# boyden/NuHTC

Hardware: AMD Instinct MI355X
Metric: tiles/sec (256x256) whole-node (higher is better)
Workload: dtype f32

## Files before the change

### include/nuhtc_hip.h

```cpp
#ifndef NUHTC_HIP_H
#define NUHTC_HIP_H

#include <stddef.h>
#include <stdint.h>

#ifdef __cplusplus
extern "C" {
#endif

#define NUHTC_ABI_VERSION 12

enum {
  NUHTC_OK = 0,
  NUHTC_E_INVALID = -1,
  NUHTC_E_HIP = -2,
  NUHTC_E_STATE = -3,
  NUHTC_E_CAPACITY = -4,
  NUHTC_E_NOTFOUND = -5
};

enum { NUHTC_CH_AS_IS = 0, NUHTC_CH_SWAP = 1 };

enum { NUHTC_PIPE_BF16_SPLIT = 0, NUHTC_PIPE_FP32 = 1 };

// ... 184 lines not shown
  const int32_t* det_off;
  const int32_t* det_counts;
  int32_t B, D, max_keep, H, W, vH, vW;
  float scale, thr;
  uint32_t* masks;
  int32_t* areas;
} nuhtc_paste_args;
int nuhtc_op_paste(nuhtc_engine* e, const nuhtc_paste_args* a, void* stream);
typedef struct nuhtc_tile_post_args {
  const float* dets;
  const int32_t* labels;
  const int32_t* areas;
  const int32_t* det_counts;
  const uint32_t* masks;
  uint8_t* keep;
  int32_t B, max_keep, H, W, vH, vW, margin, min_area;
  float thr;
} nuhtc_tile_post_args;
int nuhtc_op_tile_post(nuhtc_engine* e, const nuhtc_tile_post_args* a, void* stream);
int nuhtc_op_rpn_select(nuhtc_engine* e, const float* const out[4], const int32_t h[4], const int32_t w[4], int B, int nms_pre, int img_h, int img_w,
                        float min_size, float* cand_boxes, float* cand_scores, int32_t* cand_count, void* stream);
int nuhtc_op_nms_levels(nuhtc_engine* e, const float* boxes, const float* scores, const int32_t* group_count, int B, int G, int slot, float iou_thr,
                        int max_keep, int route, float* dets, int32_t* src, int32_t* counts, void* stream);
int nuhtc_op_build_rois(nuhtc_engine* e, const float* cc_boxes, const int32_t* cc_counts, int cc_cap, const float* rpn_dets, const int32_t* rpn_counts,
                        int rpn_cap, const float* fixed, int n_fixed, int B, int cap, float* rois, int32_t* roi_off, int32_t* roi_cnt, int32_t* total,
                        void* stream);

#define NUHTC_AP_AUTO 0
#define NUHTC_AP_GEMM 1
#define NUHTC_AP_KERNEL 2
#define NUHTC_AP_FP16 3
int nuhtc_op_attn_pool(nuhtc_engine* e, const float* F, int B, int HW, float tau, int route, float* G, void* stream);
typedef struct nuhtc_roi_feats_args {
  const float* x0;
  const float* x1;
  const float* sem;
  const float* x0sem;
  const float* G2;
  const float* G3;
  const float* rois;
  const int32_t* r_dev;
  int32_t B, cap, P;
  int32_t H[4], W[4];
  float* out;
  uint8_t* fb_flag;
  int32_t* counts;
// ... 99 lines not shown
```

### nuhtc_amd/csrc/engine.h

```cpp
#pragma once
#include <unordered_map>

#include "common.h"

struct StageGeom {
  int H, W, C, nH;
  int Hp, Wp, nW;
  int* map[2];
  int* cidx[2];
  int* ctok[2];
  int* vrow[2];
  unsigned long long* padbits[2];
  int* brow;
  int bias_row;
  float* mask;
  int* mask_any;
};

enum BlockRoute { ROUTE_PLAIN, ROUTE_A_LN, ROUTE_FUSED };

struct BlockW {
  BlockRoute route;
  float *n1g, *n1b, *relbT , *qkv_w, *qkv_b, *proj_w, *proj_b, *n2g, *n2b, *f1_w, *f1_b, *f2_w, *f2_b;
  float *qkv_wln, *qkv_bln, *f1_wln, *f1_bln;
// ... 30 lines not shown
  float *lat_w[4], *lat_b[4], *fpn_w[4], *fpn_b[4];
  float *rpn_w, *rpn_b, *rpn_hw, *rpn_hb;
  void *rpn_hf, *sem_lf[4], *sem_ef;
  float *sem_lw[4], *sem_lb[4], *sem_cw[4], *sem_cb[4], *sem_ew, *sem_eb, *sem_gw, *sem_gb;
  float *fc1_w[3], *fc1_b[3], *fc2_w[3], *fc2_b[3], *head_w[3], *head_b[3];
  float *mk_w[4], *mk_b[4], *mk_up_w, *mk_up_b, *mk_lw, *mk_lb;

  float *img, *tokA, *tokB, *xw, *qkv, *att, *hid;
  float* tok[4] = {};
  float* ln_out[4] = {};
  float *lat_wln[4] = {}, *lat_bln[4] = {};
  const uint8_t* in_tiles = nullptr;
  int in_swap = 0;
  int last_batch = 0;
  float* ln_part2 = nullptr;
  float* ln_part = nullptr;
  float *c[4], *lat[4], *x[4], *rpn[4], *semg[4];
  float *tmpA, *tmpB, *tmpR, *sem_feat, *sem_pred, *x0sem;
  PoolLevels pool{};
  double* pool_slab = nullptr;
  int roi_cap = 0;
  int cand_cap = 0;
  int* overflow = nullptr;
  int* overflow_host = nullptr;
  int32_t* export_pos = nullptr;
  int32_t* crop_size = nullptr;
  hipStream_t own = nullptr;
  hipStream_t side = nullptr;
  hipEvent_t ev_rpn = nullptr, ev_side = nullptr, ev_fpn = nullptr;
  hipStream_t side2 = nullptr;
  hipEvent_t ev_side2 = nullptr;
  struct RoiWs* rw = nullptr;
};

int dev_alloc(nuhtc_engine* e, void** p, size_t bytes);
int upload_bytes(nuhtc_engine* e, void** dst, const void* host, size_t bytes);
template <typename T>
int upload(nuhtc_engine* e, T** dst, const std::vector<T>& v) {
  return upload_bytes(e, (void**)dst, v.data(), v.size() * sizeof(T));
}
template <typename T>
int ws(nuhtc_engine* e, T** p, const char* name, std::vector<int64_t> shape, int dtype) {
  size_t n = 1;
  for (auto d : shape) n *= (size_t)d;
  int rc = dev_alloc(e, (void**)p, n * sizeof(T));
  if (rc) return rc;
// ... 32 lines not shown
```

### nuhtc_amd/csrc/proposals.h

```cpp
#pragma once
#include "common.h"

#define NMS_MAX_CAP 16384
#define NMS_MAX_GROUPS 16
#define CC_LIST_CAP 4096

struct RpnLevels {
  const float* out[4];
  int h[4], w[4], stride[4];
};

struct RpnSelParams {
  int nms_pre;
  int slot;
  float* cand_boxes;
  float* cand_scores;
  int* cand_count;
  int img_h, img_w;
  float min_size;
  unsigned* keys;
  int key_stride;
};

struct NmsParams {
  const float* boxes;
  const float* scores;
// ... 13 lines not shown
  int* out_counts;
  int* seg_start;
  int* seg_n;
  int* sorted_pos;
  unsigned long long* keepbits;
};

struct CcParams {
  const float* sem_pred;
  int h, w, img_h, img_w;
  int min_area, cap;
  unsigned char *mask_a, *mask_b, *touch;
  int* labels;
  int* stats;
  int* list;
  int* nlist;
  float* boxes;
  int* counts;
  int* overflow;
};

int launch_rpn_select(const RpnLevels& lv, const RpnSelParams& p, int B, hipStream_t s);
int launch_nms(const NmsParams& p, int B, hipStream_t s);
int launch_nms_levels(const NmsParams& p, int B, hipStream_t s);
int nms_set_attributes();
int launch_cc_mask(const CcParams& p, int B, hipStream_t s);
int launch_cc_from_mask(const CcParams& p, int B, bool open, hipStream_t s);
int launch_cc_proposals(const CcParams& p, int B, hipStream_t s);
```

### nuhtc_amd/csrc/proposals.hip

```cpp
#include "block_prims.h"
#include "common.h"
#include "proposals.h"

typedef unsigned long long u64;

__global__ __launch_bounds__(1024) void rpn_level_kernel(RpnLevels lv, RpnSelParams p) {
  __shared__ u64 keys[4096];
  __shared__ int hist[256];
  __shared__ int sc16[17];
  __shared__ unsigned s_prefix;
  __shared__ int s_need, s_cnt, s_eq;
  const int b = blockIdx.x, L = blockIdx.y;
  const int tid = threadIdx.x;
  const int h = lv.h[L], w = lv.w[L], stride = lv.stride[L];
  const int n = h * w * 3;
  const float* out = lv.out[L] + (long long)b * h * w * 32;
  const int k = p.nms_pre;
  auto score_of = [&](int idx) -> float {
    int pix = idx / 3, a = idx - pix * 3;
    float x = out[(long long)pix * 32 + a];
    return 1.0f / (1.0f + expf(-x));
  };
  int nsel;
  constexpr int RPN_KPT = 48;
// ... 459 lines not shown
  const u64* kb = p.keepbits + (long long)b * nw;
  for (int idx = tid; idx < nchunks * 64; idx += 1024) {
    if ((kb[idx >> 6] >> (idx & 63)) & 1ull) {
      const long long a = (long long)b * p.cap + idx;
      const float sc = p.scores[p.sorted_src[a]];
      const int k = atomicAdd(&s_n, 1);
      if (k < 8192) keys[k] = ((u64)desc_key_nonneg(sc) << 32) | ((u64)(unsigned)p.sorted_pos[a] << 16) | (unsigned)idx;
    }
  }
  __syncthreads();
  const int n = min(s_n, 8192);
  const int npad = next_pow2(n < 2 ? 2 : n);
  for (int i = n + tid; i < npad; i += 1024) keys[i] = ~0ull;
  __syncthreads();
  bitonic_sort_u64<1024>(keys, npad, tid);
  const int nout = min(n, p.max_keep);
  for (int k = tid; k < nout; k += 1024) {
    const int idx = (int)(keys[k] & 0xFFFFu);
    emit_det(p, b, k, p.sorted_src[(long long)b * p.cap + idx]);
  }
  if (tid == 0) p.out_counts[b] = nout;
}

int launch_nms_levels(const NmsParams& p, int B, hipStream_t s) {
  DEV_SKIP(128);
  ProfScope ps("nms", 0, 0, s);
  if (p.cap % 64 || p.cap > NMS_MAX_CAP + 64 * NMS_MAX_GROUPS || p.cap >= 65536 || p.n_groups > NMS_MAX_GROUPS || p.ids ||
      p.n_groups * p.max_keep > 8192 || !p.seg_start || !p.seg_n || !p.sorted_pos || !p.keepbits)
    return NUHTC_E_INVALID;
  size_t lds = (size_t)next_pow2(p.slot < 2 ? 2 : p.slot) * sizeof(u64);
  hipLaunchKernelGGL(nms_prepare_levels_kernel, dim3(B, p.n_groups), dim3(1024), lds, s, p);
  const int slot_chunks = (p.slot + 63) / 64;
  hipLaunchKernelGGL(nms_mask_levels_kernel, dim3(cdiv(p.n_groups * (slot_chunks * (slot_chunks + 1) / 2), 4), 1, B), dim3(256), 0, s, p);
  hipLaunchKernelGGL(nms_reduce_levels_kernel, dim3(B, p.n_groups), dim3(256), 0, s, p);
  hipLaunchKernelGGL(nms_select_kernel, dim3(B), dim3(1024), 0, s, p);
  return launched() ? 0 : NUHTC_E_HIP;
}

int nms_set_attributes() {
  hipError_t e = hipFuncSetAttribute((const void*)nms_prepare_kernel, hipFuncAttributeMaxDynamicSharedMemorySize, NMS_MAX_CAP * 8);
  if (e == hipSuccess)
    e = hipFuncSetAttribute((const void*)nms_prepare_levels_kernel, hipFuncAttributeMaxDynamicSharedMemorySize, NMS_MAX_CAP * 8);
  return e == hipSuccess ? 0 : NUHTC_E_HIP;
}

struct Gauss5 { float k[25]; };

constexpr int CCM_TW = 64, CCM_TH = 32;
__global__ __launch_bounds__(256) void cc_mask_kernel(const float* __restrict__ pred, unsigned char* __restrict__ m, int h, int w, int H,
                                                      int W, Gauss5 gk) {
  __shared__ float up[CCM_TH + 4][CCM_TW + 4 + 1];
  const int b = blockIdx.z;
  const int X0 = blockIdx.x * CCM_TW, Y0 = blockIdx.y * CCM_TH;
  const float* pb = pred + (long long)b * h * w;
  const float sy = h > 1 ? (float)(h - 1) / (float)(H - 1) : 0.f;
  const float sx = w > 1 ? (float)(w - 1) / (float)(W - 1) : 0.f;
  constexpr int NE = (CCM_TH + 4) * (CCM_TW + 4);
#pragma unroll 2
  for (int e = threadIdx.x; e < NE; e += 256) {
    int ly = e / (CCM_TW + 4), lx = e - ly * (CCM_TW + 4);
    int Y = Y0 + ly - 2, X = X0 + lx - 2;
    if (Y < 0) Y = -Y; if (Y >= H) Y = 2 * H - 2 - Y;
    if (X < 0) X = -X; if (X >= W) X = 2 * W - 2 - X;
    Y = Y < 0 ? 0 : Y; X = X < 0 ? 0 : X;
    float fy = sy * Y, fx = sx * X;
// ... 292 lines not shown
```

### nuhtc_amd/csrc/roi_engine.hip

```cpp
#include <cmath>
#include <cstring>

#include "engine.h"
#include "proposals.h"
#include "roi.h"

#define BIG_SPLIT_MAX 512
struct RoiWs {
  float *cand_boxes, *cand_scores;
  unsigned* rpn_keys;
  int rpn_key_stride;
  int* cand_count;
  float *nms_sboxes;
  int *nms_src, *nms_ntotal, *nms_seg_start, *nms_seg_n, *nms_pos;
  unsigned long long* nms_keepbits;
  unsigned long long* nms_mask;
  float* rpn_dets;
  int *rpn_src, *rpn_counts;
  int rpn_slot, rpn_cap, rpn_pow2;
  unsigned char *cc_a, *cc_b, *cc_touch;
  int *cc_labels, *cc_stats, *cc_counts, *cc_list, *cc_nlist;
  float* cc_boxes;
  float* rois;
  int *roi_off, *roi_cnt, *roi_total;
  float *G2, *G3, *ap_inv, *ap_S, *ap_Ft;
  float *feats, *h1, *h2;
  int *fb_count, *fb_list, *mid_list;
  float* big_part;
  unsigned char* fb_flag;
  float *cls[3], *reg[3];
  int total_cap;
  float *dc_boxes, *dc_scores;
  int *dc_ids, *dc_count;
  int det_cap, det_pow2;
  float* det_dets;
  int *det_src, *det_counts, *det_labels;
  float* mask_rois;
  int *det_off, *det_total;
  float *mfeat, *mtmpA, *mtmpB, *mup, *mprob;
  int mask_cap;
  unsigned* masks_own;
  int* areas_own;
// ... 58 lines not shown

static int round_up(int v, int m) { return (v + m - 1) / m * m; }
static int pow2_ge(int v) { int p = 2; while (p < v) p <<= 1; return p; }

int alloc_roi_workspace(nuhtc_engine* e) {
  const nuhtc_config& c = e->cfg;
  const int B = c.max_batch;
  const int Hn = e->Hn, Wn = e->Wn;
  RoiWs* w = new RoiWs();
  memset(w, 0, sizeof(*w));
  e->rw = w;
  int rc;
  if ((rc = nms_set_attributes())) { e->err = "hipFuncSetAttribute(nms_prepare) failed"; return rc; }
  w->rpn_slot = c.rpn_nms_pre;
  int maxc = 0;
  for (int l = 0; l < 4; ++l) maxc += std::min(c.rpn_nms_pre, e->st[l].H * e->st[l].W * 3);
  w->rpn_cap = round_up(std::max(maxc, 64), 64) + 64 * 3;
  w->rpn_pow2 = pow2_ge(maxc);
  e->roi_cap = c.max_cc_proposals + c.rpn_max_per_img;
  w->det_cap = round_up(e->roi_cap * c.num_classes, 64);
  w->det_pow2 = pow2_ge(e->roi_cap * c.num_classes);
  if (maxc > NMS_MAX_CAP || w->det_cap > NMS_MAX_CAP) { e->err = "candidate capacity exceeds NMS_MAX_CAP (reduce rpn_nms_pre / max_cc_proposals)"; return NUHTC_E_INVALID; }
  const int nmscap = std::max(w->rpn_cap, w->det_cap);
  w->rpn_key_stride = round_up(e->st[0].H * e->st[0].W * 3, 64);
  if ((rc = ws(e, &w->rpn_keys, nullptr, {B, 4, w->rpn_key_stride}, 1)) ||
      (rc = ws(e, &w->cand_boxes, "rpn_cand_boxes", {B, 4, w->rpn_slot, 4}, 0)) || (rc = ws(e, &w->cand_scores, "rpn_cand_scores", {B, 4, w->rpn_slot}, 0)) ||
      (rc = ws(e, &w->cand_count, "rpn_cand_count", {B, 4}, 1)) || (rc = ws(e, &w->nms_sboxes, nullptr, {B, nmscap, 4}, 0)) ||
      (rc = ws(e, &w->nms_src, nullptr, {B, nmscap}, 1)) || (rc = ws(e, &w->nms_ntotal, nullptr, {B}, 1)) ||
      (rc = ws(e, &w->nms_seg_start, nullptr, {B, 4}, 1)) || (rc = ws(e, &w->nms_seg_n, nullptr, {B, 4}, 1)) ||
      (rc = ws(e, &w->nms_pos, nullptr, {B, nmscap}, 1)) || (rc = ws(e, &w->nms_keepbits, nullptr, {B, nmscap / 64}, 3)) ||
      (rc = ws(e, &w->nms_mask, nullptr, {B, nmscap, nmscap / 64}, 3)) || (rc = ws(e, &w->rpn_dets, "rpn_props", {B, c.rpn_max_per_img, 5}, 0)) ||
      (rc = ws(e, &w->rpn_src, nullptr, {B, c.rpn_max_per_img}, 1)) || (rc = ws(e, &w->rpn_counts, "rpn_counts", {B}, 1)))
    return rc;
  const int64_t HW = (int64_t)Hn * Wn;
  const int ccc = std::max(c.max_cc_proposals, 1);
  if ((rc = ws(e, &w->cc_a, nullptr, {B, HW}, 2)) || (rc = ws(e, &w->cc_b, "cc_mask", {B, Hn, Wn}, 2)) || (rc = ws(e, &w->cc_touch, nullptr, {B, HW}, 2)) ||
      (rc = ws(e, &w->cc_labels, "cc_labels", {B, Hn, Wn}, 1)) || (rc = ws(e, &w->cc_stats, nullptr, {B, HW, 5}, 1)) ||
      (rc = ws(e, &w->cc_list, nullptr, {B, CC_LIST_CAP}, 1)) || (rc = ws(e, &w->cc_nlist, nullptr, {B}, 1)) ||
      (rc = ws(e, &w->cc_boxes, "cc_props", {B, ccc, 4}, 0)) || (rc = ws(e, &w->cc_counts, "cc_counts", {B}, 1)) ||
      (rc = ws(e, &e->overflow, nullptr, {4}, 1)))
    return rc;
  w->total_cap = B * e->roi_cap;
  const int T = w->total_cap;
  if ((rc = ws(e, &w->rois, "rois", {T, 5}, 0)) || (rc = ws(e, &w->roi_off, "roi_off", {B}, 1)) || (rc = ws(e, &w->roi_cnt, "roi_counts", {B}, 1)) ||
      (rc = ws(e, &w->roi_total, "roi_total", {1}, 1)) || (rc = ws(e, &w->G2, "G2", {B, e->st[2].H * e->st[2].W, 64}, 0)) ||
      (rc = ws(e, &w->G3, "G3", {B, e->st[3].H * e->st[3].W, 64}, 0)) || (rc = ws(e, &w->feats, "bbox_feats", {T, 49, 64}, 0)) ||
      (rc = ws(e, &w->h1, nullptr, {T, 256}, 0)) || (rc = ws(e, &w->h2, "h2", {T, 256}, 0)) ||
      (rc = ws(e, &w->ap_inv, nullptr, {B, e->st[2].H * e->st[2].W}, 0)) ||
      (rc = ws(e, &w->ap_S, nullptr, {B, (int64_t)e->st[2].H * e->st[2].W, (int64_t)e->st[2].H * e->st[2].W}, 0)) ||
      (rc = ws(e, &w->ap_Ft, nullptr, {B, 64, e->st[2].H * e->st[2].W}, 0)) ||
      (rc = ws(e, &w->fb_count, "roi_fallback_count", {8}, 1)) || (rc = ws(e, &w->mid_list, nullptr, {T}, 1)) || (rc = ws(e, &w->fb_list, nullptr, {T}, 1)) || (rc = ws(e, &w->fb_flag, nullptr, {T}, 2)))
    return rc;
  if ((rc = ws(e, &w->big_part, nullptr, {BIG_SPLIT_MAX, 3, 49, 64}, 0))) return rc;
  for (int k = 0; k < 3; ++k) {
// ... 50 lines not shown
}

int run_roi_path(nuhtc_engine* e, int B, const float* rois_fixed, int n_rois, int n_dets, hipStream_t s, const nuhtc_dets* out) {
  const nuhtc_config& c = e->cfg;
  RoiWs* w = e->rw;
  const int Hn = e->Hn, Wn = e->Wn;
  const bool fixed = rois_fixed != nullptr;
  if (!out || !out->boxes || !out->labels || !out->counts) FAIL(e, NUHTC_E_INVALID, "nuhtc_dets.boxes/labels/counts are required");
  if (hipMemsetAsync(e->overflow, 0, 16, s) != hipSuccess) FAIL(e, NUHTC_E_HIP, "hipMemsetAsync failed");

  if (!fixed) {
    RpnLevels lv;
    for (int l = 0; l < 4; ++l) { lv.out[l] = e->rpn[l]; lv.h[l] = e->st[l].H; lv.w[l] = e->st[l].W; lv.stride[l] = 4 << l; }
    RpnSelParams sp;
    sp.nms_pre = c.rpn_nms_pre; sp.slot = w->rpn_slot; sp.cand_boxes = w->cand_boxes; sp.cand_scores = w->cand_scores; sp.cand_count = w->cand_count; sp.keys = w->rpn_keys; sp.key_stride = w->rpn_key_stride;
    sp.img_h = e->Hv; sp.img_w = e->Wv; sp.min_size = c.rpn_min_bbox_size;
    hipStream_t s2 = e->cfg.schedule == NUHTC_SCHED_THROUGHPUT ? s : e->side;
    if (s2 != s && hipStreamWaitEvent(s2, e->ev_rpn, 0) != hipSuccess) FAIL(e, NUHTC_E_HIP, "hipStreamWaitEvent failed");
    RUN(launch_rpn_select(lv, sp, B, s2));
    NmsParams np;
    memset(&np, 0, sizeof(np));
    np.boxes = w->cand_boxes; np.scores = w->cand_scores; np.ids = nullptr; np.group_count = w->cand_count; np.n_groups = 4; np.slot = w->rpn_slot;
    np.cap = w->rpn_cap; np.cap_pow2 = w->rpn_pow2; np.iou_thr = c.rpn_nms_iou; np.max_keep = c.rpn_max_per_img;
    np.sorted_boxes = w->nms_sboxes; np.sorted_src = w->nms_src; np.n_total = w->nms_ntotal; np.mask = w->nms_mask;
    np.out_dets = w->rpn_dets; np.out_src = w->rpn_src; np.out_counts = w->rpn_counts;
    np.seg_start = w->nms_seg_start; np.seg_n = w->nms_seg_n; np.sorted_pos = w->nms_pos; np.keepbits = w->nms_keepbits;
    RUN(launch_nms_levels(np, B, s2));
    if (s2 != s && hipEventRecord(e->ev_side, s2) != hipSuccess) FAIL(e, NUHTC_E_HIP, "hipEventRecord failed");
    if (c.watershed_proposal && c.max_cc_proposals > 0) {
      CcParams cp;
      cp.sem_pred = e->sem_pred; cp.h = e->st[0].H; cp.w = e->st[0].W; cp.img_h = e->Hv; cp.img_w = e->Wv; cp.min_area = 10;    cp.cap = c.max_cc_proposals;
      cp.mask_a = w->cc_a; cp.mask_b = w->cc_b; cp.touch = w->cc_touch; cp.labels = w->cc_labels; cp.stats = w->cc_stats; cp.boxes = w->cc_boxes;
      cp.counts = w->cc_counts; cp.overflow = e->overflow; cp.list = w->cc_list; cp.nlist = w->cc_nlist;
      RUN(launch_cc_proposals(cp, B, s));
    }
  }
  const bool use_cc = !fixed && c.watershed_proposal && c.max_cc_proposals > 0;
  for (int l = 2; l < 4; ++l)
    RUN(attn_pool_table(e, e->x[l], l == 2 ? w->G2 : w->G3, B, e->st[l].H * e->st[l].W, c.att_thres, NUHTC_AP_AUTO, w->ap_inv, w->ap_S, w->ap_Ft, s));
  if (e->cfg.schedule != NUHTC_SCHED_THROUGHPUT && hipStreamWaitEvent(s, fixed ? e->ev_rpn : e->ev_side, 0) != hipSuccess) FAIL(e, NUHTC_E_HIP, "hipStreamWaitEvent failed");
  RUN(launch_build_rois(use_cc ? w->cc_boxes : nullptr, w->cc_counts, std::max(c.max_cc_proposals, 1), w->rpn_dets, w->rpn_counts, c.rpn_max_per_img,
                        rois_fixed, n_rois, w->rois, w->roi_off, w->roi_cnt, w->roi_total, B, s));
  const int Rcap = fixed ? B * n_rois : B * e->roi_cap;

  RoiFeatParams fp;
  fp.rois = w->rois; fp.r_dev = w->roi_total; fp.x0 = e->x[0]; fp.x1 = e->x[1]; fp.G2 = w->G2; fp.G3 = w->G3; fp.sem = e->sem_feat; fp.x0sem = e->x0sem;
  fp.H0 = e->st[0].H; fp.W0 = e->st[0].W; fp.H1 = e->st[1].H; fp.W1 = e->st[1].W; fp.H2 = e->st[2].H; fp.W2 = e->st[2].W; fp.H3 = e->st[3].H; fp.W3 = e->st[3].W;
// ... 259 lines not shown
  int maxn = 0;
  for (int l = 0; l < 4; ++l) {
    if (h[l] < 1 || w[l] < 1 || (long long)h[l] * w[l] * 3 > (1ll << 24)) FAIL(e, NUHTC_E_INVALID, "rpn_select op: level size out of range");
    maxn = std::max(maxn, h[l] * w[l] * 3);
  }
  HIP_CHECK(e, hipSetDevice(e->device));
  hipStream_t s = (hipStream_t)stream;
  RpnLevels lv;
  for (int l = 0; l < 4; ++l) { lv.out[l] = out[l]; lv.h[l] = h[l]; lv.w[l] = w[l]; lv.stride[l] = 4 << l; }
  DevScratch sc;
  RpnSelParams sp;
  sp.nms_pre = nms_pre; sp.slot = nms_pre; sp.cand_boxes = cand_boxes; sp.cand_scores = cand_scores; sp.cand_count = cand_count;
  sp.key_stride = round_up(maxn, 64);
  sp.keys = sc.alloc<unsigned>((size_t)B * 4 * sp.key_stride * sizeof(unsigned));
  sp.img_h = img_h; sp.img_w = img_w; sp.min_size = min_size;
  if (!sc.ok()) FAIL(e, NUHTC_E_HIP, "rpn_select op: scratch allocation failed");
  const int rc = launch_rpn_select(lv, sp, B, s);
  return op_finish(e, rc, s, "rpn_select launch refused or failed", "rpn_select kernel failed");
}

int nuhtc_op_nms_levels(nuhtc_engine* e, const float* boxes, const float* scores, const int32_t* group_count, int B, int G, int slot, float iou_thr,
                        int max_keep, int route, float* dets, int32_t* src, int32_t* counts, void* stream) {
  if (!e || !boxes || !scores || !group_count || !dets || !src || !counts) return NUHTC_E_INVALID;
  if (!e->finalized) FAIL(e, NUHTC_E_STATE, "nuhtc_op_nms_levels before finalize");
  if (B < 1 || B > 256) FAIL(e, NUHTC_E_INVALID, "nms_levels op: B out of range (1..256)");
  if (G < 1 || G > NMS_MAX_GROUPS || slot < 1 || slot > NMS_MAX_CAP || max_keep < 1 || (route != 0 && route != 1))
    FAIL(e, NUHTC_E_INVALID, "nms_levels op: G (1..16), slot (1..16384), max_keep (>= 1) or route (0, 1) out of range");
  HIP_CHECK(e, hipSetDevice(e->device));
  hipStream_t s = (hipStream_t)stream;
  std::vector<int> cnt;
  if (!read_ints(group_count, B * G, cnt, s)) FAIL(e, NUHTC_E_HIP, "nms_levels op: reading group_count failed");
  for (int c : cnt)
    if (c < 0 || c > slot) FAIL(e, NUHTC_E_INVALID, "nms_levels op: a group count exceeds slot");
  const int maxc = G * slot;
  const int cap = round_up(std::max(maxc, 64), 64) + 64 * (G - 1);
  const size_t nw = (size_t)cap / 64;
  if ((unsigned long long)B * cap * nw * 8 > (1ull << 32)) FAIL(e, NUHTC_E_INVALID, "nms_levels op: the mask matrix of this call would exceed 4 GiB");
  DevScratch sc;
  NmsParams np;
  memset(&np, 0, sizeof(np));
  np.boxes = boxes; np.scores = scores; np.ids = nullptr; np.group_count = group_count; np.n_groups = G; np.slot = slot;
  np.cap = cap; np.cap_pow2 = pow2_ge(maxc); np.iou_thr = iou_thr; np.max_keep = max_keep;
  np.out_dets = dets; np.out_src = src; np.out_counts = counts;
  struct { void** p; size_t bytes; } parts[] = {
      {(void**)&np.sorted_boxes, (size_t)B * cap * 16}, {(void**)&np.sorted_src, (size_t)B * cap * 4}, {(void**)&np.n_total, (size_t)B * 4},
      {(void**)&np.seg_start, (size_t)B * G * 4},       {(void**)&np.seg_n, (size_t)B * G * 4},        {(void**)&np.sorted_pos, (size_t)B * cap * 4},
      {(void**)&np.keepbits, (size_t)B * nw * 8},       {(void**)&np.mask, (size_t)B * cap * nw * 8}};
  int rc = 0;
  for (auto& part : parts) {
    *part.p = sc.alloc<void>(part.bytes);
    if (!sc.ok()) FAIL(e, NUHTC_E_HIP, "nms_levels op: scratch allocation failed");
    if (hipMemsetAsync(*part.p, 0xFF, part.bytes, s) != hipSuccess) rc = NUHTC_E_HIP;
  }
  if (!rc) rc = route == 0 ? launch_nms_levels(np, B, s) : launch_nms(np, B, s);
  return op_finish(e, rc, s, "nms_levels launch refused or failed (route 0: G * max_keep <= 8192; sorted-list capacity within the route's limit)",
                   "nms_levels kernel failed");
}

int nuhtc_op_build_rois(nuhtc_engine* e, const float* cc_boxes, const int32_t* cc_counts, int cc_cap, const float* rpn_dets, const int32_t* rpn_counts,
                        int rpn_cap, const float* fixed, int n_fixed, int B, int cap, float* rois, int32_t* roi_off, int32_t* roi_cnt, int32_t* total,
                        void* stream) {
  if (!e || !rois || !roi_off || !roi_cnt || !total) return NUHTC_E_INVALID;
  if (!fixed && (!rpn_dets || !rpn_counts || (cc_boxes && !cc_counts))) return NUHTC_E_INVALID;
  if (B < 1 || B > 256) FAIL(e, NUHTC_E_INVALID, "build_rois op: B out of range (1..256)");
  if (cap < 0 || cc_cap < 0 || rpn_cap < 0 || n_fixed < 0) FAIL(e, NUHTC_E_INVALID, "build_rois op: negative capacity");
  HIP_CHECK(e, hipSetDevice(e->device));
  hipStream_t s = (hipStream_t)stream;
  long long rows = (long long)B * n_fixed;
  if (!fixed) {
    std::vector<int> nr, ncc(B, 0);
    if (!read_ints(rpn_counts, B, nr, s) || (cc_boxes && !read_ints(cc_counts, B, ncc, s))) FAIL(e, NUHTC_E_HIP, "build_rois op: reading the counts failed");
    rows = 0;
    for (int b = 0; b < B; ++b) {
      if (nr[b] < 0 || nr[b] > rpn_cap || ncc[b] < 0 || ncc[b] > cc_cap) FAIL(e, NUHTC_E_INVALID, "build_rois op: a count exceeds its capacity");
      rows += nr[b] + ncc[b];
    }
  }
  if (rows > cap) FAIL(e, NUHTC_E_INVALID, "build_rois op: more rows than cap");
  const int rc = launch_build_rois(cc_boxes, cc_counts, cc_cap, rpn_dets, rpn_counts, rpn_cap, fixed, n_fixed, rois, roi_off, roi_cnt, total, B, s);
  return op_finish(e, rc, s, "build_rois launch failed", "build_rois kernel failed");
// ... 67 lines not shown
```

### nuhtc_amd/engine.py

```python
import ctypes
import os
import sys

import numpy as np
import torch

from . import hip


class HipError(RuntimeError):
    pass


class _DevView:

    def __init__(self, ptr, shape, typestr):
        self.__cuda_array_interface__ = dict(shape=tuple(int(s) for s in shape), typestr=typestr, data=(int(ptr), False),
                                             version=2, strides=None)


_TYPESTR = {0: '<f4', 1: '<i4', 2: '|u1', 3: '<u4'}
_TORCH = {0: torch.float32, 1: torch.int32, 2: torch.uint8, 3: torch.int32}


# ... 557 lines not shown
        hs = (ctypes.c_int32 * 4)(*[int(m.shape[1]) for m in maps])
        ws = (ctypes.c_int32 * 4)(*[int(m.shape[2]) for m in maps])
        self._check(self.lib.nuhtc_op_rpn_select(self.h, ptrs, hs, ws, B, K, int(img_hw[0]), int(img_hw[1]), float(min_size), cand_boxes.data_ptr(),
                                                 cand_scores.data_ptr(), cand_count.data_ptr(), self._stream()))
        return cand_boxes, cand_scores, cand_count

    def op_nms_levels(self, boxes, scores, counts, iou_thr, max_keep, route=0, dets=None, src=None):
        B, G, slot = (int(v) for v in scores.shape)
        if tuple(boxes.shape) != (B, G, slot, 4):
            raise ValueError('op_nms_levels: boxes (B, G, slot, 4) and scores (B, G, slot) expected')
        cnt = self._i32(np.asarray(counts).reshape(-1) if not isinstance(counts, torch.Tensor) else counts)
        if cnt.numel() != B * G:
            raise ValueError('op_nms_levels: counts (B, G) expected')
        K = int(max_keep)
        if dets is None:
            dets = torch.zeros(B, max(K, 1), 5, dtype=torch.float32, device=self.device)
        if src is None:
            src = torch.zeros(B, max(K, 1), dtype=torch.int32, device=self.device)
        out_counts = torch.zeros(B, dtype=torch.int32, device=self.device)
        self._check(self.lib.nuhtc_op_nms_levels(self.h, boxes.contiguous().data_ptr(), scores.contiguous().data_ptr(), cnt.contiguous().data_ptr(), B, G, slot,
                                                 float(iou_thr), K, int(route), dets.data_ptr(), src.data_ptr(), out_counts.data_ptr(), self._stream()))
        return dets, src, out_counts

    def op_build_rois(self, rpn_dets=None, rpn_counts=None, cc_boxes=None, cc_counts=None, fixed=None, B=None, rois=None, cap=None):
        dev = dict(dtype=torch.int32, device=self.device)
        if fixed is not None:
            B, nf = int(fixed.shape[0]), int(fixed.shape[1])
            need = B * nf
        else:
            B, nf = int(rpn_dets.shape[0]), 0
            rpn_counts = self._i32(rpn_counts)
            need = B * int(rpn_dets.shape[1])
            if cc_boxes is not None:
                cc_counts = self._i32(cc_counts)
                need += B * int(cc_boxes.shape[1])
        if rois is None:
            rois = torch.zeros(max(need if cap is None else int(cap), 1), 5, dtype=torch.float32, device=self.device)
        cap = int(rois.shape[0]) if cap is None else int(cap)
        r = dict(rois=rois, roi_off=torch.zeros(B, **dev), roi_cnt=torch.zeros(B, **dev), total=torch.zeros(1, **dev))
        ptr = lambda t: t.data_ptr() if t is not None else None
        self._check(self.lib.nuhtc_op_build_rois(self.h, ptr(cc_boxes), ptr(cc_counts), int(cc_boxes.shape[1]) if cc_boxes is not None else 1,
                                                 ptr(rpn_dets), ptr(rpn_counts), int(rpn_dets.shape[1]) if rpn_dets is not None else 1,
                                                 ptr(fixed), nf, B, cap, rois.data_ptr(), r['roi_off'].data_ptr(), r['roi_cnt'].data_ptr(),
                                                 r['total'].data_ptr(), self._stream()))
        return r

# ... 239 lines not shown
```

### nuhtc_amd/hip.py

```python
import ctypes
import os

HERE = os.path.dirname(os.path.abspath(__file__))
LIB_PATH = os.path.join(HERE, 'libnuhtc_hip.so')

RLE_MAX_RUNS = 15360
ABI_VERSION = 12

OK, E_INVALID, E_HIP, E_STATE, E_CAPACITY, E_NOTFOUND = 0, -1, -2, -3, -4, -5
CH_AS_IS, CH_SWAP = 0, 1
OVERLAP_MASK, OVERLAP_POLYGON = 0, 1
PIPE_BF16_SPLIT, PIPE_FP32 = 0, 1
ORDER_TOKEN, ORDER_COMPACT = 0, 1
SCHED_LATENCY, SCHED_THROUGHPUT = 0, 1
EVAL_PANNUKE, EVAL_CONIC = 0, 1
TISSUE_ALL, TISSUE_MEDIAN, TISSUE_THRESHOLD = 0, 1, 2


class Config(ctypes.Structure):
    _fields_ = [
        ('abi_version', ctypes.c_int32), ('num_classes', ctypes.c_int32),
        ('tile_h', ctypes.c_int32), ('tile_w', ctypes.c_int32), ('valid_h', ctypes.c_int32), ('valid_w', ctypes.c_int32), ('max_batch', ctypes.c_int32),
        ('scale_factor', ctypes.c_float), ('mean', ctypes.c_float * 3), ('std', ctypes.c_float * 3),
        ('rpn_nms_pre', ctypes.c_int32), ('rpn_max_per_img', ctypes.c_int32),
# ... 91 lines not shown
    ]


class StitchStore(ctypes.Structure):
    _fields_ = [
        ('n_img', ctypes.c_int32), ('cand_cap', ctypes.c_int32), ('pool_cap', ctypes.c_int32), ('work_cap', ctypes.c_int32),
        ('box', ctypes.c_void_p), ('area', ctypes.c_void_p), ('score', ctypes.c_void_p), ('label', ctypes.c_void_p), ('key', ctypes.c_void_p),
        ('off', ctypes.c_void_p), ('pool', ctypes.c_void_p), ('counters', ctypes.c_void_p), ('work', ctypes.c_void_p),
    ]


class Dets(ctypes.Structure):
    _fields_ = [('boxes', ctypes.c_void_p), ('labels', ctypes.c_void_p), ('counts', ctypes.c_void_p),
                ('masks', ctypes.c_void_p), ('areas', ctypes.c_void_p), ('keep', ctypes.c_void_p)]


EXPORTS = ['nuhtc_default_config', 'nuhtc_create', 'nuhtc_destroy', 'nuhtc_last_error', 'nuhtc_load_weight',
           'nuhtc_finalize', 'nuhtc_infer', 'nuhtc_infer_fixed_load', 'nuhtc_check', 'nuhtc_get_buffer',
           'nuhtc_op_gemm', 'nuhtc_op_gemm_split', 'nuhtc_op_roi_align', 'nuhtc_op_nms', 'nuhtc_profile_enable', 'nuhtc_profile_read', 'nuhtc_dev_knob', 'nuhtc_export_crops',
           'nuhtc_mask_contours', 'nuhtc_merge_overlap', 'nuhtc_export_kept', 'nuhtc_clock_probe', 'nuhtc_op_swin_mlp', 'nuhtc_stream', 'nuhtc_op_swin_proj_mlp', 'nuhtc_bind_host_thread',
           'nuhtc_bind_host_thread_pci', 'nuhtc_bind_host_thread_at', 'nuhtc_restore_host_thread', 'nuhtc_op_ln_gemm', 'nuhtc_op_gemm_ln_gemm', 'nuhtc_op_merge_ln_gemm', 'nuhtc_write_ring_features',
           'nuhtc_write_point_features', 'nuhtc_join_features', 'nuhtc_fill_rings', 'nuhtc_features', 'nuhtc_op_cc_mask', 'nuhtc_op_cc_proposals',
           'nuhtc_op_conv3', 'nuhtc_op_window_msa', 'nuhtc_op_bbox_tail', 'nuhtc_op_det_post', 'nuhtc_op_paste', 'nuhtc_op_tile_post',
           'nuhtc_op_rpn_select', 'nuhtc_op_nms_levels', 'nuhtc_op_build_rois', 'nuhtc_op_attn_pool', 'nuhtc_op_roi_feats',
           'nuhtc_eval_batch', 'nuhtc_op_eval_select', 'nuhtc_op_eval_pairs', 'nuhtc_op_eval_render', 'nuhtc_op_eval_joint',
           'nuhtc_stitch_gather', 'nuhtc_stitch_pairs', 'nuhtc_stitch_render', 'nuhtc_op_stitch_gather', 'nuhtc_op_stitch_pairs', 'nuhtc_op_stitch_render',
           'nuhtc_tissue_mask', 'nuhtc_points_polygon_test', 'nuhtc_grid_in_contour', 'nuhtc_rle_encode']

_lib = None


def load():
    global _lib
    if _lib is not None:
        return _lib
    if not os.path.exists(LIB_PATH):
        raise ImportError(f'{LIB_PATH} not found: the HIP extension is required (no CPU fallback exists). '
                          'Build it with `python -m nuhtc_amd.build` (hipcc, --offload-arch=gfx950).')
    import torch
    lib = ctypes.CDLL(LIB_PATH)
    vp, ci, cf = ctypes.c_void_p, ctypes.c_int, ctypes.c_float
    lib.nuhtc_default_config.argtypes = [ctypes.POINTER(Config)]
    lib.nuhtc_default_config.restype = None
    lib.nuhtc_create.argtypes = [ctypes.POINTER(Config), ci, ctypes.POINTER(vp)]
    lib.nuhtc_destroy.argtypes = [vp]
    lib.nuhtc_destroy.restype = None
    lib.nuhtc_last_error.argtypes = [vp]
# ... 6 lines not shown
    lib.nuhtc_check.argtypes = [vp, vp]
    lib.nuhtc_get_buffer.argtypes = [vp, ctypes.c_char_p, ctypes.POINTER(vp), ctypes.POINTER(ctypes.c_int64),
                                     ctypes.POINTER(ci), ctypes.POINTER(ci)]
    lib.nuhtc_op_gemm.argtypes = [vp, vp, vp, vp, vp, ci, ci, ci, ci, vp]
    lib.nuhtc_op_gemm_split.argtypes = [vp, vp, vp, vp, vp, vp, ci, ci, ci, ci, vp]
    lib.nuhtc_op_ln_gemm.argtypes = [vp, vp, ci, vp, vp, vp, vp, vp, vp, ci, ci, ci, ci, vp]
    lib.nuhtc_op_gemm_ln_gemm.argtypes = [vp, vp, vp, vp, vp, vp, vp, vp, vp, vp, vp, vp, ci, ci, ci, ci, ci, vp]
    lib.nuhtc_op_merge_ln_gemm.argtypes = [vp, vp, ci, ci, ci, ci, vp, vp, vp, vp, vp]
    lib.nuhtc_op_swin_mlp.argtypes = [vp, vp, vp, vp, vp, vp, vp, vp, vp, ci, ci, vp]
    lib.nuhtc_op_swin_proj_mlp.argtypes = [vp, vp, vp, vp, vp, vp, vp, vp, vp, vp, vp, vp, ci, ci, vp]
    lib.nuhtc_op_roi_align.argtypes = [vp, vp, ci, ci, ci, vp, ci, ci, cf, ci, vp, vp]
    lib.nuhtc_op_nms.argtypes = [vp, vp, vp, ci, cf, vp, vp, vp]
    lib.nuhtc_op_cc_mask.argtypes = [vp, vp, ci, ci, ci, ci, ci, vp, vp]
    lib.nuhtc_op_cc_proposals.argtypes = [vp, vp, ci, ci, ci, ci, ci, ci, vp, vp, vp, vp, vp, vp, vp, vp]
    lib.nuhtc_op_conv3.argtypes = [vp, ctypes.POINTER(Conv3Args), vp]
    lib.nuhtc_op_window_msa.argtypes = [vp, ctypes.POINTER(WmsaArgs), vp]
    lib.nuhtc_op_bbox_tail.argtypes = [vp, ctypes.POINTER(BboxTailArgs), vp]
    lib.nuhtc_op_det_post.argtypes = [vp, ctypes.POINTER(DetPostArgs), vp]
    lib.nuhtc_op_paste.argtypes = [vp, ctypes.POINTER(PasteArgs), vp]
    lib.nuhtc_op_tile_post.argtypes = [vp, ctypes.POINTER(TilePostArgs), vp]
    i4 = ctypes.POINTER(ctypes.c_int32)
    lib.nuhtc_op_rpn_select.argtypes = [vp, ctypes.POINTER(vp), i4, i4, ci, ci, ci, ci, cf, vp, vp, vp, vp]
    lib.nuhtc_op_nms_levels.argtypes = [vp, vp, vp, vp, ci, ci, ci, cf, ci, ci, vp, vp, vp, vp]
    lib.nuhtc_op_build_rois.argtypes = [vp, vp, vp, ci, vp, vp, ci, vp, ci, ci, ci, vp, vp, vp, vp, vp]
    lib.nuhtc_op_attn_pool.argtypes = [vp, vp, ci, ci, cf, ci, vp, vp]
    lib.nuhtc_op_roi_feats.argtypes = [vp, ctypes.POINTER(RoiFeatsArgs), vp]
    lib.nuhtc_eval_batch.argtypes = [vp, ctypes.POINTER(Dets), ci, ctypes.POINTER(EvalArgs), vp]
    lib.nuhtc_op_eval_select.argtypes = [vp, vp, ci, vp, vp, vp, ci, ci, ci, ci, cf, ctypes.c_double, vp, vp, vp, vp]
    lib.nuhtc_op_eval_pairs.argtypes = [vp, vp, vp, vp, vp, ci, ci, ci, ci, ci, ci, ci, vp, vp, vp, vp, vp]
    lib.nuhtc_op_eval_render.argtypes = [vp, vp, vp, vp, vp, ci, ci, ci, ci, ci, ci, vp, vp]
    lib.nuhtc_op_eval_joint.argtypes = [vp, vp, ci, vp, ci, ci, ci, ci, ci, ci, vp, vp, vp]
    sst = ctypes.POINTER(StitchStore)
    lib.nuhtc_stitch_gather.argtypes = [vp, ctypes.POINTER(Dets), ci, vp, cf, cf, sst, vp]
    lib.nuhtc_op_stitch_gather.argtypes = [vp, vp, vp, vp, vp, vp, ci, ci, ci, ci, cf, cf, sst, vp]
    lib.nuhtc_stitch_pairs.argtypes = lib.nuhtc_op_stitch_pairs.argtypes = [vp, sst, ci, vp, ci, vp, ci, ci, ci, ci, vp, vp, vp, vp]
    lib.nuhtc_stitch_render.argtypes = lib.nuhtc_op_stitch_render.argtypes = [vp, sst, ci, vp, ci, ci, ci, vp, vp, vp, vp]
    lib.nuhtc_mask_contours.argtypes = [vp, ctypes.POINTER(Dets), ci, ci, vp, vp, vp]
    lib.nuhtc_merge_overlap.argtypes = [ci, vp, vp, vp, vp, vp, ctypes.c_int64, ctypes.c_int64, ci, ctypes.c_double, ci, ci, ci, ci, vp, vp]
    lib.nuhtc_tissue_mask.argtypes = [ci, vp, ci, ci, ctypes.c_int64, ci, ci, ci, ci, ci, ci, vp, vp, vp, vp, vp]
    lib.nuhtc_points_polygon_test.argtypes = [ci, vp, ctypes.c_int64, vp, ctypes.c_int64, vp, vp]
    lib.nuhtc_grid_in_contour.argtypes = [ci, ci, ci, ci, ci, ci, vp, ci, ci, vp, ctypes.c_int64, vp, ctypes.c_int64, vp, ci, ci, ci, vp, vp]
    lib.nuhtc_rle_encode.argtypes = [ci, vp, vp, ci, ci, ci, ci, vp, vp, vp, ctypes.c_int64, vp, vp]
    lib.nuhtc_export_kept.argtypes = [vp, ctypes.POINTER(Dets), ci, vp, vp, ci, ci, vp, vp, vp, vp, vp, vp, vp, vp]
    lib.nuhtc_export_crops.argtypes = [vp, vp, vp, ci, vp, vp, vp, vp, ci, vp]
    lib.nuhtc_profile_enable.argtypes = [ci]
    lib.nuhtc_clock_probe.argtypes = [ci, ctypes.c_uint64, vp, vp]
# ... 101 lines not shown
```

Measured before the change: 2015.

## Fuse per-level RPN NMS into one LDS-resident kernel without global IoU mask

Adds a fused per-(image, level) NMS kernel for slots up to 4096. It sorts scores in LDS, builds only the 64x64 diagonal IoU bitmasks, and runs greedy suppression with on-the-fly IoU against the kept boxes. This replaces the separate prepare, mask and reduce kernels and drops the large global NMS mask allocation for the RPN path. The cost is a large LDS footprint per block, which limits occupancy, and a serial chunk loop with a block barrier per chunk.

```diff
diff --git a/include/nuhtc_hip.h b/include/nuhtc_hip.h
--- a/include/nuhtc_hip.h
+++ b/include/nuhtc_hip.h
@@ -230,6 +230,7 @@
                         float min_size, float* cand_boxes, float* cand_scores, int32_t* cand_count, void* stream);
 int nuhtc_op_nms_levels(nuhtc_engine* e, const float* boxes, const float* scores, const int32_t* group_count, int B, int G, int slot, float iou_thr,
                         int max_keep, int route, float* dets, int32_t* src, int32_t* counts, void* stream);
+int nuhtc_op_nms_levels_fused(nuhtc_engine* e);
 int nuhtc_op_build_rois(nuhtc_engine* e, const float* cc_boxes, const int32_t* cc_counts, int cc_cap, const float* rpn_dets, const int32_t* rpn_counts,
                         int rpn_cap, const float* fixed, int n_fixed, int B, int cap, float* rois, int32_t* roi_off, int32_t* roi_cnt, int32_t* total,
                         void* stream);
diff --git a/nuhtc_amd/csrc/engine.h b/nuhtc_amd/csrc/engine.h
--- a/nuhtc_amd/csrc/engine.h
+++ b/nuhtc_amd/csrc/engine.h
@@ -76,6 +76,7 @@
   int roi_cap = 0;
   int cand_cap = 0;
   int* overflow = nullptr;
+  int op_nms_fused = -1;
   int* overflow_host = nullptr;
   int32_t* export_pos = nullptr;
   int32_t* crop_size = nullptr;
diff --git a/nuhtc_amd/csrc/proposals.h b/nuhtc_amd/csrc/proposals.h
--- a/nuhtc_amd/csrc/proposals.h
+++ b/nuhtc_amd/csrc/proposals.h
@@ -2,6 +2,7 @@
 #include "common.h"
 
 #define NMS_MAX_CAP 16384
+#define NMS_FUSED_MAX_SLOT 4096
 #define NMS_MAX_GROUPS 16
 #define CC_LIST_CAP 4096
 
@@ -61,7 +62,8 @@
 
 int launch_rpn_select(const RpnLevels& lv, const RpnSelParams& p, int B, hipStream_t s);
 int launch_nms(const NmsParams& p, int B, hipStream_t s);
-int launch_nms_levels(const NmsParams& p, int B, hipStream_t s);
+bool nms_levels_fused(const NmsParams& p);
+int launch_nms_levels(const NmsParams& p, int B, hipStream_t s, int* fused = nullptr);
 int nms_set_attributes();
 int launch_cc_mask(const CcParams& p, int B, hipStream_t s);
 int launch_cc_from_mask(const CcParams& p, int B, bool open, hipStream_t s);
diff --git a/nuhtc_amd/csrc/proposals.hip b/nuhtc_amd/csrc/proposals.hip
--- a/nuhtc_amd/csrc/proposals.hip
+++ b/nuhtc_amd/csrc/proposals.hip
@@ -505,12 +505,124 @@
   if (tid == 0) p.out_counts[b] = nout;
 }
 
-int launch_nms_levels(const NmsParams& p, int B, hipStream_t s) {
+__host__ __device__ __forceinline__ int nms_fused_key_words(int slot) {
+  const int p2 = next_pow2(slot < 2 ? 2 : slot), s64 = (slot + 63) & ~63;
+  return p2 > s64 ? p2 : s64;
+}
+static size_t nms_fused_lds_bytes(int slot) { return (size_t)((slot + 63) & ~63) * 20 + (size_t)nms_fused_key_words(slot) * 8; }
+
+__global__ __launch_bounds__(1024) void nms_levels_fused_kernel(NmsParams p) {
+  extern __shared__ float4 sbox[];
+  __shared__ u64 removed[NMS_FUSED_MAX_SLOT / 64];
+  __shared__ u64 s_keep;
+  const int b = blockIdx.x, g = blockIdx.y, tid = threadIdx.x, lane = tid & 63, wave = tid >> 6;
+  const int slot64 = (p.slot + 63) & ~63;
+  u64* keys = reinterpret_cast<u64*>(sbox + slot64);
+  float* sarea = reinterpret_cast<float*>(keys + nms_fused_key_words(p.slot));
+  int goff[NMS_MAX_GROUPS + 1];
+  const float off = (float)g * (group_offsets_and_max(p, b, goff) + 1.0f);
+  int astart = 0, aend = 0;
+  for (int h = 0; h < p.n_groups; ++h) {
+    const int rows = (goff[h + 1] - goff[h] + 63) & ~63;
+    if (h < g) astart += rows;
+    aend += rows;
+  }
+  const int cnt = goff[g + 1] - goff[g];
+  const int npad = next_pow2(cnt < 2 ? 2 : cnt);
+  const long long base = (long long)(b * p.n_groups + g) * p.slot;
+  for (int i = tid; i < npad; i += 1024) keys[i] = i < cnt ? (((u64)desc_key_nonneg(p.scores[base + i])) << 32 | (unsigned)i) : ~0ull;
+  __syncthreads();
+  bitonic_sort_u64<1024>(keys, npad, tid);
+  for (int r = tid; r < cnt; r += 1024) {
+    const int i = (int)(keys[r] & 0xFFFFFFFFu);
+    const long long src = base + i;
+    const float* bx = p.boxes + src * 4;
+    const long long a = (long long)b * p.cap + astart + r;
+    const float4 o = make_float4(bx[0] + off, bx[1] + off, bx[2] + off, bx[3] + off);
+    sbox[r] = o;
+    sarea[r] = (o.z - o.x) * (o.w - o.y);
+    p.sorted_src[a] = (int)src;
+    p.sorted_pos[a] = goff[g] + i;
+  }
+  if (tid == 0) {
+    p.seg_start[b * p.n_groups + g] = astart;
+    p.seg_n[b * p.n_groups + g] = cnt;
+    if (g == 0) p.n_total[b] = aend;
+  }
+  const int nchunks = (cnt + 63) >> 6;
+  for (int i = tid; i < nchunks; i += 1024) removed[i] = 0;
+  __syncthreads();
+  u64* diag = keys;
+  for (int c = wave; c < nchunks; c += 16) {
+    const int ncol = min(cnt - c * 64, 64);
+    const int row = c * 64 + lane;
+    const bool live = lane < ncol;
+    const float4 a = sbox[live ? row : cnt - 1];
+    const float sa = sarea[live ? row : cnt - 1];
+    u64 bits = 0;
+    for (int j = 1; j < ncol; ++j) {
+      const float4 cj = sbox[c * 64 + j];
+      const float inter = box_inter(a, cj);
+      const bool mine = live && j > lane;
+      if (__ballot(mine && inter > 0.f) == 0) continue;
+      if (mine && inter_overlaps(inter, sa, sarea[c * 64 + j], p.iou_thr)) bits |= 1ull << j;
+    }
+    diag[row] = bits;
+  }
+  __syncthreads();
+  u64* kb_out = p.keepbits + (long long)b * (p.cap / 64) + astart / 64;
+  int kept = 0;
+  for (int c = 0; c < nchunks; ++c) {
+    if (kept >= p.max_keep) {
+      for (int i = c + tid; i < nchunks; i += 1024) kb_out[i] = 0;
+      break;
+    }
+    if (wave == 0) {
+      const u64 keep = greedy_chunk64(diag[c * 64 + lane], removed[c], p.max_keep - kept, cnt - c * 64);
+      if (lane == 0) { s_keep = keep; kb_out[c] = keep; }
+    }
+    __syncthreads();
+    const u64 keep = (u64)__builtin_amdgcn_readfirstlane((unsigned)(s_keep >> 32)) << 32 | (unsigned)__builtin_amdgcn_readfirstlane((unsigned)s_keep);
+    kept += __popcll(keep);
+    for (int w = c + 1 + wave; w < nchunks; w += 16) {
+      const int col = w * 64 + lane;
+      const u64 was = removed[w];
+      bool open = col < cnt && !((was >> lane) & 1ull);
+      const float4 cb = sbox[open ? col : w * 64];
+      const float ca = sarea[open ? col : w * 64];
+      bool hit = false;
+      u64 kb = keep;
+      while (kb && __ballot(open)) {
+        const int i = c * 64 + __ffsll((long long)kb) - 1;
+        kb &= kb - 1;
+        const float4 a = sbox[i];
+        const float inter = box_inter(a, cb);
+        const bool cand = open && inter > 0.f;
+        if (__ballot(cand) == 0) continue;
+        if (cand && inter_overlaps(inter, sarea[i], ca, p.iou_thr)) { hit = true; open = false; }
+      }
+      const u64 m = __ballot(hit);
+      if (lane == 0 && m) removed[w] = was | m;
+    }
+    __syncthreads();
+  }
+}
+
+bool nms_levels_fused(const NmsParams& p) { return p.slot <= NMS_FUSED_MAX_SLOT; }
+
+int launch_nms_levels(const NmsParams& p, int B, hipStream_t s, int* fused) {
   DEV_SKIP(128);
   ProfScope ps("nms", 0, 0, s);
   if (p.cap % 64 || p.cap > NMS_MAX_CAP + 64 * NMS_MAX_GROUPS || p.cap >= 65536 || p.n_groups > NMS_MAX_GROUPS || p.ids ||
       p.n_groups * p.max_keep > 8192 || !p.seg_start || !p.seg_n || !p.sorted_pos || !p.keepbits)
     return NUHTC_E_INVALID;
+  if (fused) *fused = nms_levels_fused(p);
+  if (nms_levels_fused(p)) {
+    hipLaunchKernelGGL(nms_levels_fused_kernel, dim3(B, p.n_groups), dim3(1024), nms_fused_lds_bytes(p.slot), s, p);
+    hipLaunchKernelGGL(nms_select_kernel, dim3(B), dim3(1024), 0, s, p);
+    return launched() ? 0 : NUHTC_E_HIP;
+  }
+  if (!p.sorted_boxes || !p.mask) return NUHTC_E_INVALID;
   size_t lds = (size_t)next_pow2(p.slot < 2 ? 2 : p.slot) * sizeof(u64);
   hipLaunchKernelGGL(nms_prepare_levels_kernel, dim3(B, p.n_groups), dim3(1024), lds, s, p);
   const int slot_chunks = (p.slot + 63) / 64;
@@ -524,6 +636,8 @@
   hipError_t e = hipFuncSetAttribute((const void*)nms_prepare_kernel, hipFuncAttributeMaxDynamicSharedMemorySize, NMS_MAX_CAP * 8);
   if (e == hipSuccess)
     e = hipFuncSetAttribute((const void*)nms_prepare_levels_kernel, hipFuncAttributeMaxDynamicSharedMemorySize, NMS_MAX_CAP * 8);
+  if (e == hipSuccess)
+    e = hipFuncSetAttribute((const void*)nms_levels_fused_kernel, hipFuncAttributeMaxDynamicSharedMemorySize, (int)nms_fused_lds_bytes(NMS_FUSED_MAX_SLOT));
   return e == hipSuccess ? 0 : NUHTC_E_HIP;
 }
 
diff --git a/nuhtc_amd/csrc/roi_engine.hip b/nuhtc_amd/csrc/roi_engine.hip
--- a/nuhtc_amd/csrc/roi_engine.hip
+++ b/nuhtc_amd/csrc/roi_engine.hip
@@ -18,6 +18,7 @@
   float* rpn_dets;
   int *rpn_src, *rpn_counts;
   int rpn_slot, rpn_cap, rpn_pow2;
+  bool rpn_fused;
   unsigned char *cc_a, *cc_b, *cc_touch;
   int *cc_labels, *cc_stats, *cc_counts, *cc_list, *cc_nlist;
   float* cc_boxes;
@@ -122,6 +123,11 @@
   w->det_pow2 = pow2_ge(e->roi_cap * c.num_classes);
   if (maxc > NMS_MAX_CAP || w->det_cap > NMS_MAX_CAP) { e->err = "candidate capacity exceeds NMS_MAX_CAP (reduce rpn_nms_pre / max_cc_proposals)"; return NUHTC_E_INVALID; }
   const int nmscap = std::max(w->rpn_cap, w->det_cap);
+  NmsParams rp;
+  memset(&rp, 0, sizeof(rp));
+  rp.slot = w->rpn_slot;
+  w->rpn_fused = nms_levels_fused(rp);
+  const int maskcap = w->rpn_fused ? w->det_cap : nmscap;
   w->rpn_key_stride = round_up(e->st[0].H * e->st[0].W * 3, 64);
   if ((rc = ws(e, &w->rpn_keys, nullptr, {B, 4, w->rpn_key_stride}, 1)) ||
       (rc = ws(e, &w->cand_boxes, "rpn_cand_boxes", {B, 4, w->rpn_slot, 4}, 0)) || (rc = ws(e, &w->cand_scores, "rpn_cand_scores", {B, 4, w->rpn_slot}, 0)) ||
@@ -129,7 +135,7 @@
       (rc = ws(e, &w->nms_src, nullptr, {B, nmscap}, 1)) || (rc = ws(e, &w->nms_ntotal, nullptr, {B}, 1)) ||
       (rc = ws(e, &w->nms_seg_start, nullptr, {B, 4}, 1)) || (rc = ws(e, &w->nms_seg_n, nullptr, {B, 4}, 1)) ||
       (rc = ws(e, &w->nms_pos, nullptr, {B, nmscap}, 1)) || (rc = ws(e, &w->nms_keepbits, nullptr, {B, nmscap / 64}, 3)) ||
-      (rc = ws(e, &w->nms_mask, nullptr, {B, nmscap, nmscap / 64}, 3)) || (rc = ws(e, &w->rpn_dets, "rpn_props", {B, c.rpn_max_per_img, 5}, 0)) ||
+      (rc = ws(e, &w->nms_mask, nullptr, {B, maskcap, maskcap / 64}, 3)) || (rc = ws(e, &w->rpn_dets, "rpn_props", {B, c.rpn_max_per_img, 5}, 0)) ||
       (rc = ws(e, &w->rpn_src, nullptr, {B, c.rpn_max_per_img}, 1)) || (rc = ws(e, &w->rpn_counts, "rpn_counts", {B}, 1)))
     return rc;
   const int64_t HW = (int64_t)Hn * Wn;
@@ -226,7 +232,7 @@
     memset(&np, 0, sizeof(np));
     np.boxes = w->cand_boxes; np.scores = w->cand_scores; np.ids = nullptr; np.group_count = w->cand_count; np.n_groups = 4; np.slot = w->rpn_slot;
     np.cap = w->rpn_cap; np.cap_pow2 = w->rpn_pow2; np.iou_thr = c.rpn_nms_iou; np.max_keep = c.rpn_max_per_img;
-    np.sorted_boxes = w->nms_sboxes; np.sorted_src = w->nms_src; np.n_total = w->nms_ntotal; np.mask = w->nms_mask;
+    np.sorted_boxes = w->nms_sboxes; np.sorted_src = w->nms_src; np.n_total = w->nms_ntotal; np.mask = w->rpn_fused ? nullptr : w->nms_mask;
     np.out_dets = w->rpn_dets; np.out_src = w->rpn_src; np.out_counts = w->rpn_counts;
     np.seg_start = w->nms_seg_start; np.seg_n = w->nms_seg_n; np.sorted_pos = w->nms_pos; np.keepbits = w->nms_keepbits;
     RUN(launch_nms_levels(np, B, s2));
@@ -532,6 +538,7 @@
 int nuhtc_op_nms_levels(nuhtc_engine* e, const float* boxes, const float* scores, const int32_t* group_count, int B, int G, int slot, float iou_thr,
                         int max_keep, int route, float* dets, int32_t* src, int32_t* counts, void* stream) {
   if (!e || !boxes || !scores || !group_count || !dets || !src || !counts) return NUHTC_E_INVALID;
+  e->op_nms_fused = -1;
   if (!e->finalized) FAIL(e, NUHTC_E_STATE, "nuhtc_op_nms_levels before finalize");
   if (B < 1 || B > 256) FAIL(e, NUHTC_E_INVALID, "nms_levels op: B out of range (1..256)");
   if (G < 1 || G > NMS_MAX_GROUPS || slot < 1 || slot > NMS_MAX_CAP || max_keep < 1 || (route != 0 && route != 1))
@@ -552,20 +559,24 @@
   np.boxes = boxes; np.scores = scores; np.ids = nullptr; np.group_count = group_count; np.n_groups = G; np.slot = slot;
   np.cap = cap; np.cap_pow2 = pow2_ge(maxc); np.iou_thr = iou_thr; np.max_keep = max_keep;
   np.out_dets = dets; np.out_src = src; np.out_counts = counts;
+  const bool no_mask = route == 0 && nms_levels_fused(np);
   struct { void** p; size_t bytes; } parts[] = {
       {(void**)&np.sorted_boxes, (size_t)B * cap * 16}, {(void**)&np.sorted_src, (size_t)B * cap * 4}, {(void**)&np.n_total, (size_t)B * 4},
       {(void**)&np.seg_start, (size_t)B * G * 4},       {(void**)&np.seg_n, (size_t)B * G * 4},        {(void**)&np.sorted_pos, (size_t)B * cap * 4},
       {(void**)&np.keepbits, (size_t)B * nw * 8},       {(void**)&np.mask, (size_t)B * cap * nw * 8}};
   int rc = 0;
   for (auto& part : parts) {
+    if (no_mask && part.p == (void**)&np.mask) continue;
     *part.p = sc.alloc<void>(part.bytes);
     if (!sc.ok()) FAIL(e, NUHTC_E_HIP, "nms_levels op: scratch allocation failed");
     if (hipMemsetAsync(*part.p, 0xFF, part.bytes, s) != hipSuccess) rc = NUHTC_E_HIP;
   }
-  if (!rc) rc = route == 0 ? launch_nms_levels(np, B, s) : launch_nms(np, B, s);
+  if (!rc) rc = route == 0 ? launch_nms_levels(np, B, s, &e->op_nms_fused) : launch_nms(np, B, s);
   return op_finish(e, rc, s, "nms_levels launch refused or failed (route 0: G * max_keep <= 8192; sorted-list capacity within the route's limit)",
                    "nms_levels kernel failed");
 }
+
+int nuhtc_op_nms_levels_fused(nuhtc_engine* e) { return e ? e->op_nms_fused : -1; }
 
 int nuhtc_op_build_rois(nuhtc_engine* e, const float* cc_boxes, const int32_t* cc_counts, int cc_cap, const float* rpn_dets, const int32_t* rpn_counts,
                         int rpn_cap, const float* fixed, int n_fixed, int B, int cap, float* rois, int32_t* roi_off, int32_t* roi_cnt, int32_t* total,
diff --git a/nuhtc_amd/engine.py b/nuhtc_amd/engine.py
--- a/nuhtc_amd/engine.py
+++ b/nuhtc_amd/engine.py
@@ -603,6 +603,9 @@
                                                  float(iou_thr), K, int(route), dets.data_ptr(), src.data_ptr(), out_counts.data_ptr(), self._stream()))
         return dets, src, out_counts
 
+    def op_nms_levels_fused(self):
+        return int(self.lib.nuhtc_op_nms_levels_fused(self.h))
+
     def op_build_rois(self, rpn_dets=None, rpn_counts=None, cc_boxes=None, cc_counts=None, fixed=None, B=None, rois=None, cap=None):
         dev = dict(dtype=torch.int32, device=self.device)
         if fixed is not None:
diff --git a/nuhtc_amd/hip.py b/nuhtc_amd/hip.py
--- a/nuhtc_amd/hip.py
+++ b/nuhtc_amd/hip.py
@@ -137,7 +137,7 @@
            'nuhtc_bind_host_thread_pci', 'nuhtc_bind_host_thread_at', 'nuhtc_restore_host_thread', 'nuhtc_op_ln_gemm', 'nuhtc_op_gemm_ln_gemm', 'nuhtc_op_merge_ln_gemm', 'nuhtc_write_ring_features',
            'nuhtc_write_point_features', 'nuhtc_join_features', 'nuhtc_fill_rings', 'nuhtc_features', 'nuhtc_op_cc_mask', 'nuhtc_op_cc_proposals',
            'nuhtc_op_conv3', 'nuhtc_op_window_msa', 'nuhtc_op_bbox_tail', 'nuhtc_op_det_post', 'nuhtc_op_paste', 'nuhtc_op_tile_post',
-           'nuhtc_op_rpn_select', 'nuhtc_op_nms_levels', 'nuhtc_op_build_rois', 'nuhtc_op_attn_pool', 'nuhtc_op_roi_feats',
+           'nuhtc_op_rpn_select', 'nuhtc_op_nms_levels', 'nuhtc_op_nms_levels_fused', 'nuhtc_op_build_rois', 'nuhtc_op_attn_pool', 'nuhtc_op_roi_feats',
            'nuhtc_eval_batch', 'nuhtc_op_eval_select', 'nuhtc_op_eval_pairs', 'nuhtc_op_eval_render', 'nuhtc_op_eval_joint',
            'nuhtc_stitch_gather', 'nuhtc_stitch_pairs', 'nuhtc_stitch_render', 'nuhtc_op_stitch_gather', 'nuhtc_op_stitch_pairs', 'nuhtc_op_stitch_render',
            'nuhtc_tissue_mask', 'nuhtc_points_polygon_test', 'nuhtc_grid_in_contour', 'nuhtc_rle_encode']
@@ -190,6 +190,7 @@
     i4 = ctypes.POINTER(ctypes.c_int32)
     lib.nuhtc_op_rpn_select.argtypes = [vp, ctypes.POINTER(vp), i4, i4, ci, ci, ci, ci, cf, vp, vp, vp, vp]
     lib.nuhtc_op_nms_levels.argtypes = [vp, vp, vp, vp, ci, ci, ci, cf, ci, ci, vp, vp, vp, vp]
+    lib.nuhtc_op_nms_levels_fused.argtypes = [vp]
     lib.nuhtc_op_build_rois.argtypes = [vp, vp, vp, ci, vp, vp, ci, vp, ci, ci, ci, vp, vp, vp, vp, vp]
     lib.nuhtc_op_attn_pool.argtypes = [vp, vp, ci, ci, cf, ci, vp, vp]
     lib.nuhtc_op_roi_feats.argtypes = [vp, ctypes.POINTER(RoiFeatsArgs), vp]
```

After: 2005. No clear change (-0.5%).
